# siyi-wind/MDViT

Hardware: AMD Instinct MI355X
Metric: 512x512 images/sec MDViT train step (fwd+bwd, two-sweep, AdamW) (higher is better)
Workload: dtype bf16x3 (fp32 storage; GEMM operands split hi+lo bf16, fp32 accumulate); 1 GPU; MDViT Sup+MLPFM train step, 4 domain(s) x bs=4 per GPU, 512x512, drop_rate=0.1 drop_path=0.1, bf16x3 GEMMs, data-parallel x1

## Files before the change

### include/mdvit_hip.h

```cpp
#ifndef MDVIT_HIP_H
#define MDVIT_HIP_H

#include <stddef.h>
#include <stdint.h>

#ifdef __cplusplus
extern "C" {
#endif

#define MDVIT_ABI_VERSION 1

enum {
    MDVIT_OK = 0,
    MDVIT_E_SHAPE = 1,
    MDVIT_E_DTYPE = 2,
    MDVIT_E_ALIGN = 3,
    MDVIT_E_WORKSPACE = 4,
    MDVIT_E_HIP = 5
};

enum { MDVIT_EPI_NONE = 0, MDVIT_EPI_GELU_DUAL = 1, MDVIT_EPI_DGELU = 2 };
enum { MDVIT_ACT_NONE = 0, MDVIT_ACT_HSWISH = 1, MDVIT_ACT_RELU = 2 };

const char* mdvit_last_error(void);
// ... 182 lines not shown
int mdvit_layernorm_fwd(const float* x, const float* gamma, const float* beta, float* y, float* mean, float* rstd,
                        int32_t M, int32_t C, int32_t groups, float eps, void* stream);
int mdvit_layernorm_bwd(const float* dy, const float* x, const float* gamma, const float* mean, const float* rstd,
                        const float* add, float* dx, float* dgamma, float* dbeta, void* ws , size_t ws_bytes,
                        int32_t M, int32_t C, int32_t groups, void* stream);
int mdvit_layernorm_bwd_masked(const float* dy, const float* x, const float* gamma, const float* mean, const float* rstd, const float* add, float* dx,
                               float* dx_masked, float* dgamma, float* dbeta, void* ws, size_t ws_bytes, int32_t M, int32_t C, int32_t groups,
                               float drop_p, uint32_t key0, uint32_t key1, const float* rowscale, int32_t rows_per_scale, const uint32_t* seed, void* stream);

int mdvit_dwconv3x3_fwd(const float* x, const float* w, const float* bias, float* y,
                        int32_t B, int32_t Hi, int32_t Wi, int32_t C, int32_t stride, int32_t add_input, void* stream);
int mdvit_dwconv3x3_bwd(const float* dy, const float* x, const float* w, float* dx, float* dw, float* dbias,
                        void* ws , size_t ws_bytes,
                        int32_t B, int32_t Hi, int32_t Wi, int32_t C, int32_t stride, int32_t add_input,
                        int32_t accumulate , void* stream);
int mdvit_gconv2_3x3_fwd(const float* skip, const float* up, const float* w, float* y,
                         int32_t B, int32_t H, int32_t W, int32_t C, void* stream);
int mdvit_gconv2_3x3_bwd(const float* dy, const float* skip, const float* up, const float* w,
                         float* dskip, float* dup, float* dw, void* ws , size_t ws_bytes,
                         int32_t B, int32_t H, int32_t W, int32_t C, int32_t accumulate , void* stream);
int mdvit_im2col3x3(const float* x, float* col, int32_t B, int32_t Hi, int32_t Wi, int32_t Cin, int32_t stride, int32_t dilation, void* stream);
int mdvit_col2im3x3(const float* dcol, float* dx, int32_t B, int32_t Hi, int32_t Wi, int32_t Cin, int32_t stride, int32_t dilation, void* stream);
int mdvit_dropout_f32(const float* x, float* y, int64_t n, float p, uint32_t key0, uint32_t key1, const uint32_t* drop_seed, void* stream);
int mdvit_stemconv_fwd(const float* img, const float* w, float* y, int32_t B, int32_t H, int32_t W, int32_t Cin, int32_t Cout, void* stream);
int mdvit_stemconv_wgrad(const float* img, const float* dy, float* dw, void* ws , size_t ws_bytes,
                         int32_t B, int32_t H, int32_t W, int32_t Cin, int32_t Cout, int32_t accumulate , void* stream);

size_t mdvit_bn_ws_bytes(int32_t M, int32_t C, int32_t groups);
int mdvit_bn_stats(const float* y, void* ws, size_t ws_bytes, float* mean, float* rstd, float* running_mean, float* running_var,
                   int64_t* num_batches_tracked, int32_t M, int32_t C, int32_t groups, int32_t per_group_affine, float eps,
                   float momentum, void* stream);
int mdvit_bn_eval_prep(const float* running_mean, const float* running_var, float* mean, float* rstd, int32_t C, float eps, void* stream);
int mdvit_bn_apply(const float* y, const float* mean, const float* rstd, const float* gamma, const float* beta, float* z,
                   int32_t M, int32_t C, int32_t groups, int32_t per_group_affine, int32_t act, float drop2d_p, uint32_t key0,
                   uint32_t key1, const uint32_t* drop_seed, int32_t rows_per_sample, void* stream);
int mdvit_bn_bwd(const float* dz, const float* y, const float* mean, const float* rstd, const float* gamma, const float* beta,
                 float* dy, float* dgamma, float* dbeta, void* ws, size_t ws_bytes, int32_t M, int32_t C, int32_t groups,
                 int32_t per_group_affine, int32_t act, int32_t training, float drop2d_p, uint32_t key0, uint32_t key1, const uint32_t* drop_seed, int32_t rows_per_sample,
                 void* stream);

size_t mdvit_bn_rowdot_ws_bytes(int32_t M, int32_t C);
int mdvit_bn_rowdot_fwd(const float* y, const float* mean, const float* rstd, const float* gamma, const float* beta, const float* w, const float* b ,
                        float* low, int32_t M, int32_t C, int32_t act, float drop2d_p, uint32_t key0, uint32_t key1, const uint32_t* drop_seed,
                        int32_t rows_per_sample, void* stream);
int mdvit_bn_rowdot_bwd(const float* g, const float* y, const float* mean, const float* rstd, const float* gamma, const float* beta, const float* w,
                        float* dy, float* dgamma, float* dbeta, float* dw, float* db , void* ws, size_t ws_bytes, int32_t M, int32_t C, int32_t act,
                        int32_t training, float drop2d_p, uint32_t key0, uint32_t key1, const uint32_t* drop_seed, int32_t rows_per_sample, void* stream);

int mdvit_upsample_fwd(const float* x, const float* base , float* y,
                       int32_t B, int32_t Hi, int32_t Wi, int32_t Ho, int32_t Wo, int32_t C, void* stream);
size_t mdvit_upsample_bwd_ws_bytes(int32_t B, int32_t Hi, int32_t Wi, int32_t Ho, int32_t Wo, int32_t C);
int mdvit_upsample_bwd(const float* dy, float* dx, void* ws, size_t ws_bytes, int32_t B, int32_t Hi, int32_t Wi, int32_t Ho, int32_t Wo,
                       int32_t C, void* stream);

int mdvit_upsample_multi_fwd(const float* const* xs, const int32_t* Hi, const int32_t* Wi, int32_t n, const float* base, float* y, int32_t B, int32_t Ho,
                             int32_t Wo, int32_t C, void* stream);
size_t mdvit_upsample_multi_bwd_ws_bytes(const int32_t* Wi, int32_t n, int32_t B, int32_t Ho, int32_t C);
int mdvit_upsample_multi_bwd(const float* dy, float* const* dxs, const int32_t* Hi, const int32_t* Wi, int32_t n, void* ws, size_t ws_bytes, int32_t B,
                             int32_t Ho, int32_t Wo, int32_t C, void* stream);

int mdvit_da_fwd(const float* label, const float* W1, const float* b1, const float* W2, const float* b2, float* a,
                 int32_t B, int32_t D, int32_t hid, int32_t C, int32_t heads, void* stream);
#define MDVIT_DA_MANY_MAX 32
typedef struct MdvitDaMany {
    int32_t n;
    int32_t hid[MDVIT_DA_MANY_MAX], C[MDVIT_DA_MANY_MAX], heads[MDVIT_DA_MANY_MAX];
    const float* W1[MDVIT_DA_MANY_MAX]; const float* b1[MDVIT_DA_MANY_MAX]; const float* W2[MDVIT_DA_MANY_MAX]; const float* b2[MDVIT_DA_MANY_MAX];
    float* a[MDVIT_DA_MANY_MAX];
} MdvitDaMany;
int mdvit_da_fwd_many(const MdvitDaMany* m, const float* label, int32_t B, int32_t D, void* stream);
typedef struct MdvitDaManyGrads {
    const float* e[MDVIT_DA_MANY_MAX];
    float* dW1[MDVIT_DA_MANY_MAX]; float* db1[MDVIT_DA_MANY_MAX]; float* dW2[MDVIT_DA_MANY_MAX]; float* db2[MDVIT_DA_MANY_MAX];
} MdvitDaManyGrads;
size_t mdvit_da_many_ws_bytes(const MdvitDaMany* m, int32_t B);
int mdvit_da_bwd_many(const MdvitDaMany* m, const MdvitDaManyGrads* g, const float* label, float scale, void* ws, size_t ws_bytes, int32_t B, int32_t D, void* stream);
size_t mdvit_da_ws_bytes(int32_t B, int32_t hid, int32_t C);
int mdvit_da_bwd(const float* label, const float* W1, const float* b1, const float* W2, const float* b2, const float* a,
                 const float* e, float scale, float* dW1, float* db1, float* dW2, float* db2, void* ws, size_t ws_bytes,
                 int32_t B, int32_t D, int32_t hid, int32_t C, int32_t heads, void* stream);

size_t mdvit_factoratt_ws_bytes(int32_t B, int32_t N, int32_t C, int32_t heads);
int mdvit_factoratt_fwd(const float* qkv, const float* w3, const float* b3, const float* w5, const float* b5,
                        const float* w7, const float* b7, const float* a, float* out, float* U, float* kmax, float* ksum, float* Mmat,
                        void* ws, size_t ws_bytes, int32_t B, int32_t H, int32_t W, int32_t C, int32_t heads,
                        int32_t s3, int32_t s5, int32_t s7, void* stream);
int mdvit_factoratt_bwd(const float* dout, const float* qkv, const float* out, const float* U,
                        const float* w3, const float* b3, const float* w5, const float* b5, const float* w7, const float* b7,
                        const float* a, const float* kmax, const float* ksum, const float* Mmat,
                        float* dqkv, float* e, float* dw3, float* db3, float* dw5, float* db5, float* dw7, float* db7,
                        void* ws, size_t ws_bytes, int32_t B, int32_t H, int32_t W, int32_t C, int32_t heads,
                        int32_t s3, int32_t s5, int32_t s7, void* stream);
int mdvit_factoratt_wgrad(const float* qkv, void* ws, size_t ws_bytes, float* dw3, float* db3, float* dw5, float* db5,
                          float* dw7, float* db7, int32_t B, int32_t H, int32_t W, int32_t C, int32_t heads,
                          int32_t s3, int32_t s5, int32_t s7, int32_t accumulate, void* stream);

int mdvit_seg_losses_fwd(const float* out, const float* aux, const float* label, double* sums, float* losses, int64_t n, void* stream);
int mdvit_seg_losses_sums(const float* out, const float* aux, const float* label, double* sums, int64_t n, void* stream);
int mdvit_seg_losses_final(const double* sums, float* losses, int64_t n_total, int32_t has_aux, void* stream);
int mdvit_seg_losses_bwd(const float* out, const float* aux, const float* label, const double* sums, const float* g,
                         float* dout, float* daux, int64_t n, float dice_gain, void* stream);
int mdvit_seg_losses_bwd3(const float* out, const float* aux, const float* label, const double* sums, const float* g0, const float* g1, const float* g2,
                          float* dout, float* daux, int64_t n, float dice_gain, void* stream);
int mdvit_seg_losses_groups_sums(const float* out, const float* aux, const float* label, double* sums, int64_t n, int32_t G, void* stream);
int mdvit_seg_losses_groups_final(const double* sums, float* losses, float* per_group, int64_t n_total, int32_t has_aux, int32_t G, void* stream);
int mdvit_seg_losses_groups_bwd(const float* out, const float* aux, const float* label, const double* sums, const float* g0, const float* g1, const float* g2,
// ... 69 lines not shown
```

### mdvit_amd/_lib.py

```python
from __future__ import annotations

import ctypes as C
import os
import re
from typing import List

_HERE = os.path.dirname(os.path.abspath(__file__))
LIB_PATH = os.environ.get("MDVIT_HIP_LIB") or os.path.join(_HERE, "lib", "libmdvit_hip.so")
HEADER_PATH = os.path.join(_HERE, "..", "include", "mdvit_hip.h")

EPI_NONE, EPI_GELU_DUAL, EPI_DGELU = 0, 1, 2
ACT_NONE, ACT_HSWISH, ACT_RELU = 0, 1, 2

f32p = C.c_void_p
vp = C.c_void_p
i32 = C.c_int32
i64 = C.c_int64
u32 = C.c_uint32
f32 = C.c_float


class GemmDesc(C.Structure):
    _fields_ = [
        ("A", vp), ("B", vp), ("C", vp), ("C2", vp),
# ... 145 lines not shown
    "mdvit_patchify": [vp, vp, i32, i32, i32, i32, i32, vp],
    "mdvit_dropout2d": [vp, vp, i32, i64, i32, f32, u32, u32, vp, vp],
    "mdvit_sdpa_fwd": [vp, vp, vp, vp, i32, i32, i32, i32, vp],
    "mdvit_sdpa_bwd": [vp, vp, vp, vp, vp, vp, vp, vp, i32, i32, i32, i32, vp],
    "mdvit_sdpa_mfma_fwd": [vp, vp, vp, vp, i32, i32, i32, i32, vp],
    "mdvit_sdpa_mfma_bwd": [vp, vp, vp, vp, vp, vp, vp, vp, i32, i32, i32, i32, vp],
    "mdvit_structure_weight": [vp, vp, vp, i32, i32, i32, vp],
    "mdvit_structure_loss_fwd": [vp, vp, vp, vp, vp, i32, i64, vp],
    "mdvit_structure_loss_bwd": [vp, vp, vp, vp, vp, vp, i32, i64, vp],
    "mdvit_split_planes": [vp, i64, vp, i64, i64, i64, i32, i32, vp],
    "mdvit_split_planes_many": [vp, i32, i32, i32, vp],
    "mdvit_split_planes_t": [vp, i64, vp, i64, i64, i32, i32, i32, i32, vp],
    "mdvit_event_create": [C.POINTER(vp)],
    "mdvit_event_destroy": [vp],
    "mdvit_event_elapsed_ms": [vp, vp, C.POINTER(f32)],
    "mdvit_timing_arm": [vp, vp],
    "mdvit_gemm_f32": [C.POINTER(GemmDesc), vp],
    "mdvit_gemm_plan": [C.POINTER(GemmDesc), C.POINTER(i32), C.POINTER(i32), C.POINTER(i32)],
    "mdvit_gemm_force_plan": [i32, i32],
    "mdvit_conv_weight_relayout": [vp, vp, i32, i32, i32, vp],
    "mdvit_conv_weight_relayout_many": [vp, i32, i32, vp],
    "mdvit_gemm_kernel_name": [vp, C.c_char_p, i32],
    "mdvit_gemm_tn_config": [i32, i32, i32],
    "mdvit_gemm_tn_grid_order": [i32],
    "mdvit_transpose_f32": [vp, i64, vp, i32, i32, vp],
    "mdvit_mlp_bwd_dgrad_f32": [vp, vp, vp, vp, vp, vp, vp, vp, i32, i32, i32, f32, u32, u32, vp, vp],
    "mdvit_mlp_fwd_f32": [vp, vp, vp, vp, vp, vp, vp, i32, vp, vp, i32, i32, i32, f32, u32, u32, u32, u32, vp, vp],
    "mdvit_transpose_many": [vp, i32, i32, vp],
    "mdvit_rowdot_fwd": [vp, i64, vp, vp, vp, i32, i32, i32, vp],
    "mdvit_rowdot_bwd": [vp, i64, vp, vp, vp, i64, vp, vp, vp, C.c_size_t, i32, i32, vp],
    "mdvit_colsum_f32": [vp, i64, vp, vp, vp, C.c_size_t, i32, i32, f32, u32, u32, vp, i32, i32, vp, vp],
    "mdvit_layernorm_fwd": [vp, vp, vp, vp, vp, vp, i32, i32, i32, f32, vp],
    "mdvit_layernorm_bwd": [vp, vp, vp, vp, vp, vp, vp, vp, vp, vp, C.c_size_t, i32, i32, i32, vp],
    "mdvit_layernorm_bwd_masked": [vp, vp, vp, vp, vp, vp, vp, vp, vp, vp, vp, C.c_size_t, i32, i32, i32, f32, u32, u32, vp, i32, vp, vp],
    "mdvit_dwconv3x3_fwd": [vp, vp, vp, vp, i32, i32, i32, i32, i32, i32, vp],
    "mdvit_dwconv3x3_bwd": [vp, vp, vp, vp, vp, vp, vp, C.c_size_t, i32, i32, i32, i32, i32, i32, i32, vp],
    "mdvit_gconv2_3x3_fwd": [vp, vp, vp, vp, i32, i32, i32, i32, vp],
    "mdvit_gconv2_3x3_bwd": [vp, vp, vp, vp, vp, vp, vp, vp, C.c_size_t, i32, i32, i32, i32, i32, vp],
    "mdvit_im2col3x3": [vp, vp, i32, i32, i32, i32, i32, i32, vp],
    "mdvit_col2im3x3": [vp, vp, i32, i32, i32, i32, i32, i32, vp],
    "mdvit_dropout_f32": [vp, vp, i64, f32, u32, u32, vp, vp],
    "mdvit_stemconv_fwd": [vp, vp, vp, i32, i32, i32, i32, i32, vp],
    "mdvit_stemconv_wgrad": [vp, vp, vp, vp, C.c_size_t, i32, i32, i32, i32, i32, i32, vp],
    "mdvit_bn_rowdot_fwd": [vp, vp, vp, vp, vp, vp, vp, vp, i32, i32, i32, f32, u32, u32, vp, i32, vp],
    "mdvit_bn_rowdot_bwd": [vp, vp, vp, vp, vp, vp, vp, vp, vp, vp, vp, vp, vp, C.c_size_t, i32, i32, i32, i32, f32, u32, u32, vp, i32, vp],
    "mdvit_bn_stats": [vp, vp, C.c_size_t, vp, vp, vp, vp, vp, i32, i32, i32, i32, f32, f32, vp],
    "mdvit_bn_eval_prep": [vp, vp, vp, vp, i32, f32, vp],
    "mdvit_bn_apply": [vp, vp, vp, vp, vp, vp, i32, i32, i32, i32, i32, f32, u32, u32, vp, i32, vp],
    "mdvit_bn_bwd": [vp, vp, vp, vp, vp, vp, vp, vp, vp, vp, C.c_size_t, i32, i32, i32, i32, i32, i32, f32, u32, u32, vp, i32, vp],
    "mdvit_upsample_multi_fwd": [vp, vp, vp, i32, vp, vp, i32, i32, i32, i32, vp],
    "mdvit_upsample_multi_bwd": [vp, vp, vp, vp, i32, vp, C.c_size_t, i32, i32, i32, i32, vp],
    "mdvit_upsample_fwd": [vp, vp, vp, i32, i32, i32, i32, i32, i32, vp],
    "mdvit_upsample_bwd": [vp, vp, vp, C.c_size_t, i32, i32, i32, i32, i32, i32, vp],
    "mdvit_da_fwd": [vp, vp, vp, vp, vp, vp, i32, i32, i32, i32, i32, vp],
    "mdvit_da_bwd": [vp] * 7 + [f32] + [vp] * 4 + [vp, C.c_size_t] + [i32] * 5 + [vp],
    "mdvit_factoratt_fwd": [vp] * 13 + [vp, C.c_size_t] + [i32] * 8 + [vp],
    "mdvit_factoratt_wgrad": [vp, vp, C.c_size_t] + [vp] * 6 + [i32] * 9 + [vp],
    "mdvit_factoratt_bwd": [vp] * 22 + [vp, C.c_size_t] + [i32] * 8 + [vp],
    "mdvit_seg_losses_fwd": [vp, vp, vp, vp, vp, i64, vp],
    "mdvit_adamw_step": [vp, i32, i32, vp, vp, f32, f32, f32, f32, i32, vp],
    "mdvit_seg_metrics": [vp, vp, vp, vp, vp, i64, vp],
    "mdvit_image_normalize_u8": [vp, vp, i32, i32, i32, vp],
    "mdvit_augment_normalize_u8": [vp, vp, vp, vp, vp, vp, i32, i32, i32, vp],
    "mdvit_augment_probe_taps": [f32, f32, i32, i32, C.POINTER(i32), C.POINTER(f32)],
    "mdvit_seg_losses_sums": [vp, vp, vp, vp, i64, vp],
    "mdvit_seg_losses_final": [vp, vp, i64, i32, vp],
    "mdvit_seg_losses_bwd": [vp, vp, vp, vp, vp, vp, vp, i64, f32, vp],
    "mdvit_seg_losses_bwd3": [vp, vp, vp, vp, vp, vp, vp, vp, vp, i64, f32, vp],
    "mdvit_seg_losses_groups_sums": [vp, vp, vp, vp, i64, i32, vp],
    "mdvit_seg_losses_groups_final": [vp, vp, vp, i64, i32, i32, vp],
    "mdvit_seg_losses_groups_bwd": [vp, vp, vp, vp, vp, vp, vp, vp, vp, i64, i32, f32, vp],
    "mdvit_se_adapter_fwd": [C.POINTER(SeAdapterDesc), vp, vp, vp, vp, C.c_size_t, vp],
    "mdvit_se_adapter_bwd": [C.POINTER(SeAdapterDesc)] + [vp] * 10 + [vp, C.c_size_t, vp],
}

_lib = None


class MdvitHipError(RuntimeError):
    pass


def declared_symbols() -> List[str]:
    with open(HEADER_PATH) as f:
        text = f.read()
    text = re.sub(r"/\*.*?\*/", "", text, flags=re.S)
    return sorted(set(re.findall(r"\b(mdvit_[a-z0-9_]+)\s*\(", text)))


_on_load = []


def on_load(fn):
    if _lib is not None:
        fn(_lib)
    else:
        _on_load.append(fn)


def load():
    global _lib
    if _lib is not None:
        return _lib
    if not os.path.exists(LIB_PATH):
        raise MdvitHipError(
            f"{LIB_PATH} is missing: build it with `python -m mdvit_amd.build` (hipcc, gfx950). "
# ... 71 lines not shown
```

### mdvit_amd/csrc/conv.hip

```cpp
#include "common.h"
#include "conv_tile.h"

namespace {

__device__ __forceinline__ float4 f4_fma(float4 a, float4 w, float4 acc) {
    acc.x = fmaf(a.x, w.x, acc.x); acc.y = fmaf(a.y, w.y, acc.y); acc.z = fmaf(a.z, w.z, acc.z); acc.w = fmaf(a.w, w.w, acc.w);
    return acc;
}
__device__ __forceinline__ float4 f4_add(float4 a, float4 b) { return make_float4(a.x + b.x, a.y + b.y, a.z + b.z, a.w + b.w); }

__global__ __launch_bounds__(256) void dwconv3x3_fwd_kernel(const float* __restrict__ x, const float* __restrict__ w,
                                                            const float* __restrict__ bias, float* __restrict__ y,
                                                            int B, int Hi, int Wi, int C, int stride, int add_input) {
    extern __shared__ float s_w[];
    for (int i = threadIdx.x; i < 9 * C; i += blockDim.x) { const int c = i / 9, t = i % 9; s_w[t * C + c] = w[i]; }
    __syncthreads();
    const int Ho = (Hi - 1) / stride + 1, Wo = (Wi - 1) / stride + 1, QC = C >> 2;
    const long total = (long)B * Ho * Wo * QC;
    for (long e = (long)blockIdx.x * blockDim.x + threadIdx.x; e < total; e += (long)gridDim.x * blockDim.x) {
        const int c = (int)(e % QC) * 4;
        long tkn = e / QC;
        const int wo = (int)(tkn % Wo); tkn /= Wo;
        const int ho = (int)(tkn % Ho);
        const int b = (int)(tkn / Ho);
// ... 701 lines not shown
        if (j >= p.Wi[0]) { j -= p.Wi[0]; src = 1; if (j >= p.Wi[1]) { j -= p.Wi[1]; src = 2; } }
        const int Wi = p.Wi[src];
        const float sc = (float)Wi / (float)Wo;
        int lo, hi;
        out_range(j, Wi, Wo, lo, hi);
        float4 acc = make_float4(0.f, 0.f, 0.f, 0.f);
        const float* base = dy + o * Wo * C + c;
#pragma unroll 4
        for (int t = lo; t < hi; ++t) {
            int i0, i1; float l;
            bilin_src(t, Wi, sc, i0, i1, l);
            const float wgt = (i0 == j ? 1.f - l : 0.f) + (i1 == j ? l : 0.f);
            const float4 g = *reinterpret_cast<const float4*>(base + (long)t * C);
            acc.x = fmaf(wgt, g.x, acc.x); acc.y = fmaf(wgt, g.y, acc.y); acc.z = fmaf(wgt, g.z, acc.z); acc.w = fmaf(wgt, g.w, acc.w);
        }
        float* dsts[3] = {p.d[0], p.d[1], p.d[2]};
        *reinterpret_cast<float4*>(dsts[src] + (o * Wi + j) * C + c) = acc;
    }
}

__global__ __launch_bounds__(256) void upsample_multi_bwd_w_lds_kernel(UpMulti p, const float* __restrict__ dy, int Wo, int C) {
    extern __shared__ __attribute__((aligned(16))) float s_row[];
    const long o = blockIdx.x;
    const int c0 = blockIdx.y * 32;
    const float* src = dy + o * Wo * C + c0;
    for (int e = threadIdx.x; e < Wo * 8; e += 256) {
        const int t = e >> 3, q = e & 7;
        *reinterpret_cast<float4*>(s_row + t * 32 + 4 * q) = *reinterpret_cast<const float4*>(src + (long)t * C + 4 * q);
    }
    __syncthreads();
    const int Wsum = p.Wi[0] + (p.n > 1 ? p.Wi[1] : 0) + (p.n > 2 ? p.Wi[2] : 0);
    float* dsts[3] = {p.d[0], p.d[1], p.d[2]};
    for (int e = threadIdx.x; e < Wsum * 8; e += 256) {
        const int q = e & 7;
        int j = e >> 3, sidx = 0;
        if (j >= p.Wi[0]) { j -= p.Wi[0]; sidx = 1; if (j >= p.Wi[1]) { j -= p.Wi[1]; sidx = 2; } }
        const int Wi = p.Wi[sidx];
        const float sc = (float)Wi / (float)Wo;
        int lo, hi;
        out_range(j, Wi, Wo, lo, hi);
        float4 acc = make_float4(0.f, 0.f, 0.f, 0.f);
#pragma unroll 4
        for (int t = lo; t < hi; ++t) {
            int i0, i1; float l;
            bilin_src(t, Wi, sc, i0, i1, l);
            const float wgt = (i0 == j ? 1.f - l : 0.f) + (i1 == j ? l : 0.f);
            const float4 g = *reinterpret_cast<const float4*>(s_row + t * 32 + 4 * q);
            acc.x = fmaf(wgt, g.x, acc.x); acc.y = fmaf(wgt, g.y, acc.y); acc.z = fmaf(wgt, g.z, acc.z); acc.w = fmaf(wgt, g.w, acc.w);
        }
        *reinterpret_cast<float4*>(dsts[sidx] + (o * Wi + j) * C + c0 + 4 * q) = acc;
    }
}

__global__ __launch_bounds__(256) void dropout_kernel(const float* __restrict__ x, float* __restrict__ y, long n4, uint32_t k0, uint32_t k1,
                                                      const uint32_t* __restrict__ seed, uint32_t thresh, float inv_keep) {
    const uint32_t k0e = k0 ^ (seed ? seed[0] : 0u), k1e = k1 + (seed ? seed[1] : 0u);
    for (long i = (long)blockIdx.x * blockDim.x + threadIdx.x; i < n4; i += (long)gridDim.x * blockDim.x) {
        const float4 v = *reinterpret_cast<const float4*>(x + 4 * i);
        const float4 d = mdvit_drop_scale4(k0e, k1e, (uint32_t)(4 * i), thresh, inv_keep);
        *reinterpret_cast<float4*>(y + 4 * i) = make_float4(v.x * d.x, v.y * d.y, v.z * d.z, v.w * d.w);
    }
}

inline int ew_grid(long total) { return (int)min((total + 255) / 256, 16384L); }

}

extern "C" int mdvit_dwconv3x3_fwd(const float* x, const float* w, const float* bias, float* y, int32_t B, int32_t Hi, int32_t Wi,
                                   int32_t C, int32_t stride, int32_t add_input, void* stream) {
    MDVIT_CHECK_ARG(B > 0 && Hi > 0 && Wi > 0 && C > 0 && C % 4 == 0 && C <= 4096, MDVIT_E_SHAPE, "dwconv3x3_fwd: bad shape B=%d H=%d W=%d C=%d", B, Hi, Wi, C);
    MDVIT_CHECK_ARG(stride == 1 || stride == 2, MDVIT_E_SHAPE, "dwconv3x3_fwd: stride must be 1 or 2");
    MDVIT_CHECK_ARG(!(add_input && stride != 1), MDVIT_E_SHAPE, "dwconv3x3_fwd: add_input needs stride 1");
    const int Ho = (Hi - 1) / stride + 1, Wo = (Wi - 1) / stride + 1;
    if (stride == 1) {
        launch_conv_tile<3, false>(x, (long)C, 0, w, bias, y, (long)C, 0, CtGeom{B, Hi, Wi}, C, (hipStream_t)stream, add_input);
        MDVIT_LAUNCH_CHECK();
        return MDVIT_OK;
    }
    const long total = (long)B * Ho * Wo * C / 4;
    hipLaunchKernelGGL(dwconv3x3_fwd_kernel, dim3(ew_grid(total)), dim3(256), sizeof(float) * 9 * C, (hipStream_t)stream,
                       x, w, bias, y, B, Hi, Wi, C, stride, add_input);
    MDVIT_LAUNCH_CHECK();
    return MDVIT_OK;
}

extern "C" int mdvit_dwconv3x3_bwd(const float* dy, const float* x, const float* w, float* dx, float* dw, float* dbias, void* ws, size_t ws_bytes,
                                   int32_t B, int32_t Hi, int32_t Wi, int32_t C, int32_t stride, int32_t add_input, int32_t accumulate,
                                   void* stream) {
    hipStream_t s = (hipStream_t)stream;
    MDVIT_CHECK_ARG(B > 0 && Hi > 0 && Wi > 0 && C > 0 && C % 4 == 0 && C <= 1024, MDVIT_E_SHAPE, "dwconv3x3_bwd: bad shape B=%d H=%d W=%d C=%d", B, Hi, Wi, C);
    MDVIT_CHECK_ARG(stride == 1 || stride == 2, MDVIT_E_SHAPE, "dwconv3x3_bwd: stride must be 1 or 2");
    const int Ho = (Hi - 1) / stride + 1, Wo = (Wi - 1) / stride + 1;
    if (stride == 1) {
        const CtGeom cg{B, Hi, Wi};
        if (dx) launch_conv_tile<3, true>(dy, (long)C, 0, w, nullptr, dx, (long)C, 0, cg, C, s, add_input);
        if (dw) {
            int tpb; long nblk;
            conv_wgrad_plan(cg, C, tpb, nblk);
            MDVIT_CHECK_PARTIALS_WS(ws, ws_bytes, nblk, CT_CL * 10, "dwconv3x3_bwd");
            const int rc = launch_conv_tile_wgrad<3>(dy, (long)C, 0, x, (long)C, 0, dw, dbias, (float*)ws, cg, C, s, accumulate);
            if (rc != MDVIT_OK) return rc;
        }
        MDVIT_LAUNCH_CHECK();
        return MDVIT_OK;
    }
    if (dx) {
// ... 78 lines not shown
    MDVIT_CHECK_ARG(n > 0 && n % 4 == 0 && n < (1L << 32) && p >= 0.f && p < 1.f, MDVIT_E_SHAPE, "dropout: need 0 < n < 2^32, n %% 4 == 0, 0 <= p < 1 (n=%ld p=%g)", (long)n, p);
    MDVIT_CHECK_ARG(aligned16(x) && aligned16(y), MDVIT_E_ALIGN, "dropout: 16-byte aligned buffers");
    hipLaunchKernelGGL(dropout_kernel, dim3(ew_grid(n / 4)), dim3(256), 0, (hipStream_t)stream, x, y, (long)(n / 4), key0, key1, drop_seed,
                       mdvit_drop_thresh(p), 1.f / (1.f - p));
    MDVIT_LAUNCH_CHECK();
    return MDVIT_OK;
}

extern "C" int mdvit_stemconv_fwd(const float* img, const float* w, float* y, int32_t B, int32_t H, int32_t W, int32_t Cin, int32_t Cout, void* stream) {
    MDVIT_CHECK_ARG(Cin == 3, MDVIT_E_SHAPE, "stemconv_fwd: only in_chans == 3 is built (got %d)", Cin);
    MDVIT_CHECK_ARG(B > 0 && H > 0 && W > 0 && Cout > 0 && Cout % 4 == 0 && Cout <= 256, MDVIT_E_SHAPE, "stemconv_fwd: bad shape");
    const int Ho = (H - 1) / 2 + 1, Wo = (W - 1) / 2 + 1;
    static const bool px32 = [] { const char* e = getenv("MDVIT_STEM_FWD32"); return !(e && e[0] == '0'); }();
    if (px32 && Cout == 32)
        hipLaunchKernelGGL((stemconv_fwd32_kernel<3>), dim3((int)min(((long)B * Ho * Wo + 127) / 128, 8192L)), dim3(256), 0, (hipStream_t)stream, img, w, y, B, H, W);
    else
        hipLaunchKernelGGL((stemconv_fwd_kernel<3>), dim3(ew_grid((long)B * Ho * Wo * Cout / 4)), dim3(256), sizeof(float) * 27 * Cout, (hipStream_t)stream,
                           img, w, y, B, H, W, Cout);
    MDVIT_LAUNCH_CHECK();
    return MDVIT_OK;
}

extern "C" int mdvit_stemconv_wgrad(const float* img, const float* dy, float* dw, void* ws, size_t ws_bytes, int32_t B, int32_t H, int32_t W,
                                    int32_t Cin, int32_t Cout, int32_t accumulate, void* stream) {
    hipStream_t s = (hipStream_t)stream;
    MDVIT_CHECK_ARG(Cin == 3, MDVIT_E_SHAPE, "stemconv_wgrad: only in_chans == 3 is built (got %d)", Cin);
    MDVIT_CHECK_ARG(B > 0 && H > 0 && W > 0 && Cout > 0 && Cout <= 256, MDVIT_E_SHAPE, "stemconv_wgrad: bad shape");
    const int Ho = (H - 1) / 2 + 1, Wo = (W - 1) / 2 + 1;
    const long npix = (long)B * Ho * Wo;
    int ppb = (int)max(64L, (npix + 2047) / 2048);
    const int nblk = cdiv(npix, ppb);
    MDVIT_CHECK_PARTIALS_WS(ws, ws_bytes, nblk, 27 * Cout, "stemconv_wgrad");
    static const bool mfma = [] { const char* e = getenv("MDVIT_STEM_WGRAD_MFMA"); return !(e && e[0] == '0'); }();
    if (mfma && Cout % 32 == 0) {
        ppb = (int)max(128L, (npix + 1023) / 1024);
        const int nb2 = cdiv(npix, ppb);
        hipLaunchKernelGGL((stemconv_wgrad_mfma_kernel<3>), dim3(nb2), dim3(256), 0, s, img, dy, (float*)ws, B, H, W, Cout, ppb);
        MDVIT_LAUNCH_CHECK();
        return mdvit_reduce_partials((const float*)ws, nb2, 27L * Cout, 27 * Cout, dw, 0, nullptr, accumulate, s);
    }
    hipLaunchKernelGGL((stemconv_wgrad_kernel<3>), dim3(nblk), dim3(256), sizeof(float) * 27 * Cout, s, img, dy, (float*)ws, B, H, W, Cout, ppb);
    MDVIT_LAUNCH_CHECK();
    return mdvit_reduce_partials((const float*)ws, nblk, 27L * Cout, 27 * Cout, dw, 0, nullptr, accumulate, s);
}

extern "C" int mdvit_upsample_fwd(const float* x, const float* base, float* y, int32_t B, int32_t Hi, int32_t Wi, int32_t Ho, int32_t Wo, int32_t C, void* stream) {
    MDVIT_CHECK_ARG(B > 0 && Hi > 0 && Wi > 0 && Ho > 0 && Wo > 0 && C > 0, MDVIT_E_SHAPE, "upsample_fwd: bad shape");
    const long total = (long)B * Ho * Wo * ((C & 3) == 0 ? C / 4 : C);
    hipLaunchKernelGGL(upsample_fwd_kernel, dim3(ew_grid(total)), dim3(256), 0, (hipStream_t)stream, x, base, y, B, Hi, Wi, Ho, Wo, C);
    MDVIT_LAUNCH_CHECK();
    return MDVIT_OK;
}

extern "C" size_t mdvit_upsample_bwd_ws_bytes(int32_t B, int32_t Hi, int32_t Wi, int32_t Ho, int32_t Wo, int32_t C) {
    if (B <= 0 || Hi <= 0 || Wi <= 0 || Ho <= 0 || Wo <= 0 || C <= 0) return 0;
    return sizeof(float) * (size_t)B * Ho * Wi * C;
}

extern "C" int mdvit_upsample_bwd(const float* dy, float* dx, void* ws, size_t ws_bytes, int32_t B, int32_t Hi, int32_t Wi, int32_t Ho, int32_t Wo,
                                  int32_t C, void* stream) {
    hipStream_t s = (hipStream_t)stream;
    MDVIT_CHECK_ARG(B > 0 && Hi > 0 && Wi > 0 && Ho > 0 && Wo > 0 && C > 0, MDVIT_E_SHAPE, "upsample_bwd: bad shape");
    MDVIT_CHECK_ARG(ws != nullptr && ws_bytes >= mdvit_upsample_bwd_ws_bytes(B, Hi, Wi, Ho, Wo, C), MDVIT_E_WORKSPACE,
                    "upsample_bwd: workspace too small (mdvit_upsample_bwd_ws_bytes)");
    float* tmp = (float*)ws;
    const int vec = (C & 3) == 0 && aligned16(dy) && aligned16(dx) && aligned16(tmp);
    const long cq = vec ? C / 4 : C;
    {
        const long total = (long)B * Ho * Wi * cq;
        hipLaunchKernelGGL((upsample_bwd_pass_kernel<true>), dim3(ew_grid(total)), dim3(256), 0, s, dy, tmp, (long)B * Ho, Wi, Wo, cq, vec);
    }
    {
        const long total = (long)B * Hi * Wi * cq;
        hipLaunchKernelGGL((upsample_bwd_pass_kernel<false>), dim3(ew_grid(total)), dim3(256), 0, s, tmp, dx, (long)B, Hi, Ho, (long)Wi * cq, vec);
    }
    MDVIT_LAUNCH_CHECK();
    return MDVIT_OK;
}

extern "C" int mdvit_upsample_multi_fwd(const float* const* xs, const int32_t* Hi, const int32_t* Wi, int32_t n, const float* base, float* y, int32_t B, int32_t Ho,
                                        int32_t Wo, int32_t C, void* stream) {
    MDVIT_CHECK_ARG(n >= 1 && n <= 3 && B > 0 && Ho > 0 && Wo > 0 && C > 0 && C % 4 == 0, MDVIT_E_SHAPE, "upsample_multi_fwd: 1..3 sources, C %% 4 == 0 (n=%d C=%d)", n, C);
    UpMulti p; memset(&p, 0, sizeof(p));
    p.n = n;
    for (int i = 0; i < n; ++i) {
        MDVIT_CHECK_ARG(xs[i] && Hi[i] > 0 && Wi[i] > 0 && aligned16(xs[i]), MDVIT_E_SHAPE, "upsample_multi_fwd: bad source %d", i);
        p.x[i] = xs[i]; p.Hi[i] = Hi[i]; p.Wi[i] = Wi[i];
    }
    MDVIT_CHECK_ARG(aligned16(y) && (!base || aligned16(base)), MDVIT_E_ALIGN, "upsample_multi_fwd: y / base must be 16-byte aligned");
    {
        bool ok = Ho % UT_H == 0 && Wo % UT_W == 0 && C % UT_C == 0 && (long)(Ho / UT_H) * (Wo / UT_W) < (1L << 30) && C / UT_C < 65536 && B < 65536;
        int pool = 0;
        for (int i = 0; i < n && ok; ++i) {
            const int fh = Ho / Hi[i], fw = Wo / Wi[i];
            ok = Ho % Hi[i] == 0 && Wo % Wi[i] == 0 && fh >= 2 && fw >= 2 && fh <= 16 && fw <= 16 && (fh & (fh - 1)) == 0 && (fw & (fw - 1)) == 0;
            if (ok) pool += (UT_H / fh + 2) * (UT_W / fw + 2);
        }
        if (ok && pool <= UT_POOL) {
            hipLaunchKernelGGL(upsample_multi_tile_kernel, dim3((Ho / UT_H) * (Wo / UT_W), C / UT_C, B), dim3(256), 0, (hipStream_t)stream, p, base, y, Ho, Wo, C);
            MDVIT_LAUNCH_CHECK();
            return MDVIT_OK;
        }
    }
    MDVIT_CHECK_ARG((long)Wo * (C / 4) < (1L << 30), MDVIT_E_SHAPE, "upsample_multi_fwd: output row too long");
    const long nunits = (long)B * Ho * (((long)Wo * (C / 4) + 1023) >> 10);
    hipLaunchKernelGGL(upsample_multi_fwd_kernel, dim3((unsigned)min(nunits, 16384L)), dim3(256), 0, (hipStream_t)stream, p, base, y, B, Ho, Wo, C);
    MDVIT_LAUNCH_CHECK();
    return MDVIT_OK;
}

extern "C" size_t mdvit_upsample_multi_bwd_ws_bytes(const int32_t* Wi, int32_t n, int32_t B, int32_t Ho, int32_t C) {
    size_t t = 0;
    for (int i = 0; i < n && i < 3; ++i) t += (size_t)B * Ho * Wi[i] * C;
    return sizeof(float) * t;
}

extern "C" int mdvit_upsample_multi_bwd(const float* dy, float* const* dxs, const int32_t* Hi, const int32_t* Wi, int32_t n, void* ws, size_t ws_bytes, int32_t B,
                                        int32_t Ho, int32_t Wo, int32_t C, void* stream) {
    hipStream_t s = (hipStream_t)stream;
    MDVIT_CHECK_ARG(n >= 1 && n <= 3 && B > 0 && Ho > 0 && Wo > 0 && C > 0 && C % 4 == 0, MDVIT_E_SHAPE, "upsample_multi_bwd: 1..3 sources, C %% 4 == 0 (n=%d C=%d)", n, C);
    MDVIT_CHECK_ARG(ws && ws_bytes >= mdvit_upsample_multi_bwd_ws_bytes(Wi, n, B, Ho, C) && aligned16(ws) && aligned16(dy), MDVIT_E_WORKSPACE,
                    "upsample_multi_bwd: workspace too small (mdvit_upsample_multi_bwd_ws_bytes)");
    UpMulti p; memset(&p, 0, sizeof(p));
    p.n = n;
    float* t = (float*)ws;
    int wsum = 0;
    for (int i = 0; i < n; ++i) {
        MDVIT_CHECK_ARG(dxs[i] && Hi[i] > 0 && Wi[i] > 0 && aligned16(dxs[i]), MDVIT_E_SHAPE, "upsample_multi_bwd: bad source %d", i);
        p.Hi[i] = Hi[i]; p.Wi[i] = Wi[i]; p.d[i] = t;
        t += (size_t)B * Ho * Wi[i] * C;
        wsum += Wi[i];
    }
    const long cq = C / 4;
    const int bpr = (int)cdiv((long)wsum * cq, 256L);
    MDVIT_CHECK_ARG((long)B * Ho * bpr < (1L << 31), MDVIT_E_SHAPE, "upsample_multi_bwd: too many workgroups");
    if (C % 32 == 0 && Wo <= 384 && (long)B * Ho < (1L << 31) && C / 32 <= 65535)
        hipLaunchKernelGGL(upsample_multi_bwd_w_lds_kernel, dim3((unsigned)((long)B * Ho), C / 32), dim3(256), sizeof(float) * Wo * 32, s, p, dy, Wo, C);
    else
        hipLaunchKernelGGL(upsample_multi_bwd_w_kernel, dim3((unsigned)((long)B * Ho * bpr)), dim3(256), 0, s, p, dy, (long)B * Ho, Wo, C, bpr);
    for (int i = 0; i < n; ++i)
        hipLaunchKernelGGL((upsample_bwd_pass_kernel<false>), dim3(ew_grid((long)B * Hi[i] * Wi[i] * cq)), dim3(256), 0, s, p.d[i], dxs[i], (long)B, Hi[i], Ho,
                           (long)Wi[i] * cq, 1);
    MDVIT_LAUNCH_CHECK();
    return MDVIT_OK;
}
```

### mdvit_amd/ops.py

```python
from __future__ import annotations

import ctypes as C
import itertools
import os
import weakref
from typing import Optional, Tuple

import torch

from . import _lib
from ._lib import GemmDesc, call

_key_counter = itertools.count(1)
_POISON = os.environ.get("MDVIT_POISON", "0") == "1"


def _empty(*a, **k):
    t = torch.empty(*a, **k)
    if _POISON and t.is_floating_point():
        t.fill_(float("nan"))
    return t


def _empty_like(x):
# ... 1931 lines not shown
            off += n
        return tuple(out)

    @staticmethod
    def backward(ctx, *gs):
        if all(g is None for g in gs):
            return None, None
        ref = next(g for g in gs if g is not None)
        parts = [g if g is not None else torch.zeros((ctx.rows, n), device=ref.device, dtype=ref.dtype) for g, n in zip(gs, ctx.sizes)]
        return torch.cat(parts, 1), None


class _CatChannels(torch.autograd.Function):

    @staticmethod
    def forward(ctx, a, b):
        ctx.set_materialize_grads(False)
        ctx.sizes = (a.shape[-1], b.shape[-1])
        return torch.cat([a, b], dim=-1)

    @staticmethod
    def backward(ctx, g):
        if g is None:
            return None, None
        c0, _c1 = ctx.sizes
        return (g[..., :c0].contiguous() if ctx.needs_input_grad[0] else None), (g[..., c0:].contiguous() if ctx.needs_input_grad[1] else None)


def cat_channels(a, b):
    return _CatChannels.apply(_c(a), _c(b))


def split_cols(W, sizes):
    assert W.dim() == 2 and sum(sizes) == W.shape[1]
    return _SplitCols.apply(W, tuple(int(n) for n in sizes))


def split_groups(x, groups: int):
    if groups == 1:
        return (x,)
    assert x.shape[0] % groups == 0
    return _SplitGroups.apply(_c(x), int(groups))


def bn_act(y, gamma, beta, running_mean, running_var, nbt, training, act, eps=1e-5, momentum=0.1, drop2d_p=0.0):
    rows_per_sample = y.numel() // (y.shape[0] * y.shape[-1])
    groups = _bn_groups if (training or gamma.dim() == 2) else 1
    if groups > 1 and y.shape[0] % groups:
        raise ValueError(f"bn_groups({groups}) needs a batch that is a multiple of it, got {y.shape[0]}")
    return _BNAct.apply(_c(y), _c(gamma), _c(beta), running_mean, running_var, nbt, bool(training), float(eps), float(momentum),
                        int(act), float(drop2d_p), int(rows_per_sample), int(groups))


class _Upsample(torch.autograd.Function):
    @staticmethod
    def forward(ctx, x, Ho, Wo, base):
        ctx.set_materialize_grads(False)
        _chk(x, base)
        B, H, W_, Cn = x.shape
        y = _empty((B, Ho, Wo, Cn), device=x.device, dtype=torch.float32)
        call("mdvit_upsample_fwd", _p(x), _p(base), _p(y), B, H, W_, Ho, Wo, Cn, _stream())
        ctx.meta = (B, H, W_, Ho, Wo, Cn, base is not None)
        return y

    @staticmethod
    def backward(ctx, g):
        if g is None:
            return (None,) * 4
        B, H, W_, Ho, Wo, Cn, has_base = ctx.meta
        g = _c(g)
        dx = _empty((B, H, W_, Cn), device=g.device, dtype=torch.float32)
        wsb = _lib.load().mdvit_upsample_bwd_ws_bytes(B, H, W_, Ho, Wo, Cn)
        ws = _empty((wsb // 4,), device=g.device, dtype=torch.float32)
        call("mdvit_upsample_bwd", _p(g), _p(dx), _p(ws), wsb, B, H, W_, Ho, Wo, Cn, _stream())
        return dx, None, None, (g if has_base else None)


def upsample_bilinear(x, Ho, Wo, base=None):
    if base is None and x.shape[1] == Ho and x.shape[2] == Wo:
        return x
    return _Upsample.apply(_c(x), int(Ho), int(Wo), None if base is None else _c(base))


class _UpsampleSum(torch.autograd.Function):

    @staticmethod
    def forward(ctx, base, Ho, Wo, *xs):
        ctx.set_materialize_grads(False)
        _chk(base, *xs)
        B, _, _, Cn = xs[0].shape
        n = len(xs)
        y = _empty((B, Ho, Wo, Cn), device=xs[0].device, dtype=torch.float32)
        ptrs = (C.c_void_p * n)(*[x.data_ptr() for x in xs])
        Hi = (C.c_int32 * n)(*[x.shape[1] for x in xs])
        Wi = (C.c_int32 * n)(*[x.shape[2] for x in xs])
        call("mdvit_upsample_multi_fwd", ptrs, Hi, Wi, n, _p(base), _p(y), B, Ho, Wo, Cn, _stream())
        ctx.meta = (B, Ho, Wo, Cn, [(x.shape[1], x.shape[2]) for x in xs], base is not None)
        return y

    @staticmethod
    def backward(ctx, g):
        B, Ho, Wo, Cn, dims, has_base = ctx.meta
        if g is None:
            return (None,) * (3 + len(dims))
        g = _c(g)
        n = len(dims)
# ... 817 lines not shown
```

Before: 516.3 images/s.

## Fuse bilinear upsample backward width and height passes into single kernels

Adds a fused multi-source upsample backward kernel that streams dy rows through double-buffered LDS, applies precomputed width weights and accumulates height contributions in registers, writing dx directly instead of going through a workspace and a second height pass. Also adds a simple fused single-source kernel for small-channel upsample backward. Both apply only to even integer scale factors and are on by default, with an env switch to disable. The goal is to remove the intermediate workspace round trip and extra launches, at the cost of complex indexing and possible lower occupancy from LDS use.

```diff
diff --git a/include/mdvit_hip.h b/include/mdvit_hip.h
--- a/include/mdvit_hip.h
+++ b/include/mdvit_hip.h
@@ -258,6 +258,7 @@
 size_t mdvit_upsample_bwd_ws_bytes(int32_t B, int32_t Hi, int32_t Wi, int32_t Ho, int32_t Wo, int32_t C);
 int mdvit_upsample_bwd(const float* dy, float* dx, void* ws, size_t ws_bytes, int32_t B, int32_t Hi, int32_t Wi, int32_t Ho, int32_t Wo,
                        int32_t C, void* stream);
+int mdvit_upsample_bwd_config(int32_t fused);
 
 int mdvit_upsample_multi_fwd(const float* const* xs, const int32_t* Hi, const int32_t* Wi, int32_t n, const float* base, float* y, int32_t B, int32_t Ho,
                              int32_t Wo, int32_t C, void* stream);
diff --git a/mdvit_amd/_lib.py b/mdvit_amd/_lib.py
--- a/mdvit_amd/_lib.py
+++ b/mdvit_amd/_lib.py
@@ -221,6 +221,7 @@
     "mdvit_upsample_multi_bwd": [vp, vp, vp, vp, i32, vp, C.c_size_t, i32, i32, i32, i32, vp],
     "mdvit_upsample_fwd": [vp, vp, vp, i32, i32, i32, i32, i32, i32, vp],
     "mdvit_upsample_bwd": [vp, vp, vp, C.c_size_t, i32, i32, i32, i32, i32, i32, vp],
+    "mdvit_upsample_bwd_config": [i32],
     "mdvit_da_fwd": [vp, vp, vp, vp, vp, vp, i32, i32, i32, i32, i32, vp],
     "mdvit_da_bwd": [vp] * 7 + [f32] + [vp] * 4 + [vp, C.c_size_t] + [i32] * 5 + [vp],
     "mdvit_factoratt_fwd": [vp] * 13 + [vp, C.c_size_t] + [i32] * 8 + [vp],
diff --git a/mdvit_amd/csrc/conv.hip b/mdvit_amd/csrc/conv.hip
--- a/mdvit_amd/csrc/conv.hip
+++ b/mdvit_amd/csrc/conv.hip
@@ -777,6 +777,206 @@
     }
 }
 
+constexpr int UA_R = 16;
+constexpr int UA_ITEMS = 4;
+constexpr int UA_PAD = 8;
+constexpr int UA_HT = UA_R + 32;
+
+template <int NPF>
+__global__ __launch_bounds__(256) void upsample_multi_bwd_fused_kernel(UpMulti p, const float* __restrict__ dy, int Ho, int Wo, int C) {
+    extern __shared__ __attribute__((aligned(16))) float s_rows[];
+    const int rowf = (Wo + 2 * UA_PAD) * 32;
+    float4* s_ht = reinterpret_cast<float4*>(s_rows + 2 * rowf);
+    float* s_wt = reinterpret_cast<float*>(s_ht + UA_HT * 3);
+    const int c0 = blockIdx.x * 32, b = blockIdx.z;
+    const int R0 = blockIdx.y * UA_R, R1 = min(R0 + UA_R, Ho);
+    int ob = Ho, oe = 0;
+    for (int i = 0; i < p.n; ++i) {
+        const int s = Ho / p.Hi[i];
+        const int rf = (R0 + s - 1) / s, re = min(p.Hi[i], (R1 + s - 1) / s);
+        if (rf < re) { ob = min(ob, max(0, s * rf - s / 2)); oe = max(oe, min(Ho, s * (re - 1) + 3 * s / 2)); }
+    }
+    if (ob >= oe) return;
+    for (int e = threadIdx.x; e < (oe - ob) * p.n; e += 256) {
+        const int o = ob + e / p.n, i = e % p.n;
+        const int Hi = i == 0 ? p.Hi[0] : i == 1 ? p.Hi[1] : p.Hi[2];
+        const int s = Ho / Hi, rh = (o + s / 2) / s;
+        int i0, i1; float l;
+        bilin_src(o, Hi, (float)Hi / (float)Ho, i0, i1, l);
+        const int rE = (rh & 1) ? rh - 1 : rh, rO = (rh & 1) ? rh : rh - 1;
+        const float wE = (i0 == rE ? 1.f - l : 0.f) + (i1 == rE ? l : 0.f);
+        const float wO = (i0 == rO ? 1.f - l : 0.f) + (i1 == rO ? l : 0.f);
+        int ev = 0;
+        if ((o + 1 + s / 2) % s == 0) {
+            const int rd = rh - 1, rf = (R0 + s - 1) / s, re = min(Hi, (R1 + s - 1) / s);
+            ev = 2 * (rd + 2) + (rd >= rf && rd < re ? 1 : 0);
+        }
+        s_ht[(o - ob) * 3 + i] = make_float4(wE, wO, __int_as_float(ev), 0.f);
+    }
+    {
+        int wbase = 0;
+        for (int i = 0; i < p.n; ++i) {
+            const int Wi = p.Wi[i], s = Wo / Wi;
+            const float sc = (float)Wi / (float)Wo;
+            for (int e = threadIdx.x; e < Wi * 2 * s; e += 256) {
+                const int j = e / (2 * s), t = s * j - s / 2 + e % (2 * s);
+                float wgt = 0.f;
+                if (t >= 0 && t < Wo) {
+                    int i0, i1; float l;
+                    bilin_src(t, Wi, sc, i0, i1, l);
+                    wgt = (i0 == j ? 1.f - l : 0.f) + (i1 == j ? l : 0.f);
+                }
+                s_wt[wbase + e] = wgt;
+            }
+            wbase += Wi * 2 * s;
+        }
+    }
+    for (int e = threadIdx.x; e < 2 * 2 * UA_PAD * 8; e += 256) {
+        const int buf = e / (2 * UA_PAD * 8), r = e % (2 * UA_PAD * 8), px = r >> 3;
+        *reinterpret_cast<float4*>(s_rows + buf * rowf + (px < UA_PAD ? px : Wo + px) * 32 + 4 * (r & 7)) = make_float4(0.f, 0.f, 0.f, 0.f);
+    }
+    const int Wsum = p.Wi[0] + (p.n > 1 ? p.Wi[1] : 0) + (p.n > 2 ? p.Wi[2] : 0);
+    const int q = threadIdx.x & 7;
+    int it_src[UA_ITEMS], it_t0[UA_ITEMS], it_s2[UA_ITEMS], it_wo[UA_ITEMS];
+    long it_rs[UA_ITEMS];
+    float* it_dx[UA_ITEMS];
+    float4 aE[UA_ITEMS], aO[UA_ITEMS];
+#pragma unroll
+    for (int k = 0; k < UA_ITEMS; ++k) {
+        const int e = threadIdx.x + 256 * k;
+        int j = e >> 3, sidx = 0, wbase = 0;
+        if (j >= p.Wi[0]) {
+            j -= p.Wi[0]; sidx = 1; wbase = 2 * Wo;
+            if (j >= p.Wi[1]) { j -= p.Wi[1]; sidx = 2; wbase = 4 * Wo; }
+        }
+        if (e >= Wsum * 8) { sidx = -1; j = 0; }
+        const int Hi = sidx <= 0 ? p.Hi[0] : sidx == 1 ? p.Hi[1] : p.Hi[2];
+        const int Wi = sidx <= 0 ? p.Wi[0] : sidx == 1 ? p.Wi[1] : p.Wi[2];
+        float* dx = sidx <= 0 ? p.d[0] : sidx == 1 ? p.d[1] : p.d[2];
+        const int s = Wo / Wi;
+        it_src[k] = sidx;
+        it_t0[k] = s * j - s / 2 + UA_PAD; it_s2[k] = 2 * s;
+        it_wo[k] = wbase + j * 2 * s;
+        it_rs[k] = (long)Wi * C;
+        it_dx[k] = dx + ((long)b * Hi * Wi + j) * C + c0 + 4 * q;
+        aE[k] = make_float4(0.f, 0.f, 0.f, 0.f); aO[k] = make_float4(0.f, 0.f, 0.f, 0.f);
+    }
+    const float* src = dy + (long)b * Ho * Wo * C + c0;
+    typedef float f4v __attribute__((ext_vector_type(4)));
+    f4v pfa[NPF], pfb[NPF];
+#pragma unroll
+    for (int u = 0; u < NPF; ++u) {
+        const int e = threadIdx.x + 256 * u;
+        if (e < Wo * 8) *reinterpret_cast<float4*>(s_rows + (UA_PAD + (e >> 3)) * 32 + 4 * (e & 7)) = *reinterpret_cast<const float4*>(src + ((long)ob * Wo + (e >> 3)) * C + 4 * (e & 7));
+    }
+#define UA_FMA(wv, gv) acc.x = fmaf(wv, gv.x, acc.x); acc.y = fmaf(wv, gv.y, acc.y); acc.z = fmaf(wv, gv.z, acc.z); acc.w = fmaf(wv, gv.w, acc.w);
+#define UA_STEP(o, cur, ld, st) { \
+        { \
+        _Pragma("unroll") \
+            for (int u = 0; u < NPF; ++u) { \
+                const int e = min((int)threadIdx.x + 256 * u, Wo * 8 - 1); \
+                ld[u] = *reinterpret_cast<const f4v*>(src + ((long)min(o + 2, oe - 1) * Wo + (e >> 3)) * C + 4 * (e & 7)); \
+            } \
+        } \
+        const float* s_row = s_rows + cur * rowf + 4 * q; \
+        _Pragma("unroll") \
+        for (int k = 0; k < UA_ITEMS; ++k) { \
+            if (it_src[k] < 0 || (o) >= oe) continue; \
+            const float* wt = s_wt + it_wo[k]; \
+            const float* sr = s_row + it_t0[k] * 32; \
+            float4 acc = make_float4(0.f, 0.f, 0.f, 0.f); \
+            int u = 0; \
+            for (; u + 8 <= it_s2[k]; u += 8) { \
+                const float4 w0 = *reinterpret_cast<const float4*>(wt + u), w1 = *reinterpret_cast<const float4*>(wt + u + 4); \
+                const float4 g0 = *reinterpret_cast<const float4*>(sr + (u + 0) * 32), g1 = *reinterpret_cast<const float4*>(sr + (u + 1) * 32); \
+                const float4 g2 = *reinterpret_cast<const float4*>(sr + (u + 2) * 32), g3 = *reinterpret_cast<const float4*>(sr + (u + 3) * 32); \
+                const float4 g4 = *reinterpret_cast<const float4*>(sr + (u + 4) * 32), g5 = *reinterpret_cast<const float4*>(sr + (u + 5) * 32); \
+                const float4 g6 = *reinterpret_cast<const float4*>(sr + (u + 6) * 32), g7 = *reinterpret_cast<const float4*>(sr + (u + 7) * 32); \
+                UA_FMA(w0.x, g0) UA_FMA(w0.y, g1) UA_FMA(w0.z, g2) UA_FMA(w0.w, g3) UA_FMA(w1.x, g4) UA_FMA(w1.y, g5) UA_FMA(w1.z, g6) UA_FMA(w1.w, g7) \
+            } \
+            if (u < it_s2[k]) { \
+                const float4 w0 = *reinterpret_cast<const float4*>(wt + u); \
+                const float4 g0 = *reinterpret_cast<const float4*>(sr + (u + 0) * 32), g1 = *reinterpret_cast<const float4*>(sr + (u + 1) * 32); \
+                const float4 g2 = *reinterpret_cast<const float4*>(sr + (u + 2) * 32), g3 = *reinterpret_cast<const float4*>(sr + (u + 3) * 32); \
+                UA_FMA(w0.x, g0) UA_FMA(w0.y, g1) UA_FMA(w0.z, g2) UA_FMA(w0.w, g3) \
+            } \
+            const float4 h = s_ht[(o - ob) * 3 + it_src[k]]; \
+            aE[k].x = fmaf(h.x, acc.x, aE[k].x); aE[k].y = fmaf(h.x, acc.y, aE[k].y); aE[k].z = fmaf(h.x, acc.z, aE[k].z); aE[k].w = fmaf(h.x, acc.w, aE[k].w); \
+            aO[k].x = fmaf(h.y, acc.x, aO[k].x); aO[k].y = fmaf(h.y, acc.y, aO[k].y); aO[k].z = fmaf(h.y, acc.z, aO[k].z); aO[k].w = fmaf(h.y, acc.w, aO[k].w); \
+            const int ev = __float_as_int(h.z); \
+            if (ev) { \
+                const int rd = (ev >> 1) - 2; \
+                float* d = it_dx[k] + rd * it_rs[k]; \
+                if (rd & 1) { if (ev & 1) *reinterpret_cast<float4*>(d) = aO[k]; aO[k] = make_float4(0.f, 0.f, 0.f, 0.f); } \
+                else        { if (ev & 1) *reinterpret_cast<float4*>(d) = aE[k]; aE[k] = make_float4(0.f, 0.f, 0.f, 0.f); } \
+            } \
+        } \
+        if (o + 1 < oe) { \
+            float* nxt = s_rows + (cur ^ 1) * rowf + UA_PAD * 32; \
+        _Pragma("unroll") \
+            for (int u = 0; u < NPF; ++u) { \
+                const int e = threadIdx.x + 256 * u; \
+                if (e < Wo * 8) *reinterpret_cast<f4v*>(nxt + (e >> 3) * 32 + 4 * (e & 7)) = st[u]; \
+            } \
+        } \
+        __syncthreads(); \
+    }
+#pragma unroll
+    for (int u = 0; u < NPF; ++u) {
+        const int e = min((int)threadIdx.x + 256 * u, Wo * 8 - 1);
+        pfb[u] = *reinterpret_cast<const f4v*>(src + ((long)min(ob + 1, Ho - 1) * Wo + (e >> 3)) * C + 4 * (e & 7));
+    }
+    __syncthreads();
+    for (int o = ob; o < oe; o += 2) {
+        UA_STEP(o, 0, pfa, pfb)
+        UA_STEP(o + 1, 1, pfb, pfa)
+    }
+#undef UA_STEP
+#undef UA_FMA
+#pragma unroll
+    for (int k = 0; k < UA_ITEMS; ++k) {
+        if (it_src[k] < 0) continue;
+        const int Hi = it_src[k] == 0 ? p.Hi[0] : it_src[k] == 1 ? p.Hi[1] : p.Hi[2];
+        const int s = Ho / Hi, rh = (oe + s / 2) / s;
+        const int rf = (R0 + s - 1) / s, re = min(Hi, (R1 + s - 1) / s);
+        const int rE = (rh & 1) ? rh - 1 : rh, rO = (rh & 1) ? rh : rh - 1;
+        if (rE >= rf && rE < re) *reinterpret_cast<float4*>(it_dx[k] + rE * it_rs[k]) = aE[k];
+        if (rO >= rf && rO < re) *reinterpret_cast<float4*>(it_dx[k] + rO * it_rs[k]) = aO[k];
+    }
+}
+
+__global__ __launch_bounds__(256) void upsample_bwd_fused_kernel(const float* __restrict__ dy, float* __restrict__ dx, int B, int Hi, int Wi, int Ho, int Wo, int C) {
+    const float sch = (float)Hi / (float)Ho, scw = (float)Wi / (float)Wo;
+    const long total = (long)B * Hi * Wi * C;
+    for (long e = (long)blockIdx.x * blockDim.x + threadIdx.x; e < total; e += (long)gridDim.x * blockDim.x) {
+        const int c = (int)(e % C);
+        long r = e / C;
+        const int j = (int)(r % Wi); r /= Wi;
+        const int i = (int)(r % Hi);
+        const long b = r / Hi;
+        int lo_h, hi_h, lo_w, hi_w;
+        out_range(i, Hi, Ho, lo_h, hi_h);
+        out_range(j, Wi, Wo, lo_w, hi_w);
+        float acc = 0.f;
+        for (int o = lo_h; o < hi_h; ++o) {
+            const float* base = dy + (b * Ho + o) * Wo * C + c;
+            float tw = 0.f;
+#pragma unroll 4
+            for (int t = lo_w; t < hi_w; ++t) {
+                int i0, i1; float l;
+                bilin_src(t, Wi, scw, i0, i1, l);
+                const float wgt = (i0 == j ? 1.f - l : 0.f) + (i1 == j ? l : 0.f);
+                tw = fmaf(wgt, base[(long)t * C], tw);
+            }
+            int i0, i1; float l;
+            bilin_src(o, Hi, sch, i0, i1, l);
+            const float wgt = (i0 == i ? 1.f - l : 0.f) + (i1 == i ? l : 0.f);
+            acc = fmaf(wgt, tw, acc);
+        }
+        dx[e] = acc;
+    }
+}
+
 __global__ __launch_bounds__(256) void dropout_kernel(const float* __restrict__ x, float* __restrict__ y, long n4, uint32_t k0, uint32_t k1,
                                                       const uint32_t* __restrict__ seed, uint32_t thresh, float inv_keep) {
     const uint32_t k0e = k0 ^ (seed ? seed[0] : 0u), k1e = k1 + (seed ? seed[1] : 0u);
@@ -961,6 +1161,13 @@
     return MDVIT_OK;
 }
 
+static int g_upsample_bwd_fused = 1;
+extern "C" int mdvit_upsample_bwd_config(int32_t fused) {
+    g_upsample_bwd_fused = fused != 0;
+    return MDVIT_OK;
+}
+static bool even_factor(int n_in, int n_out) { return n_out % n_in == 0 && ((n_out / n_in) & 1) == 0 && n_out / n_in <= 16; }
+
 extern "C" size_t mdvit_upsample_bwd_ws_bytes(int32_t B, int32_t Hi, int32_t Wi, int32_t Ho, int32_t Wo, int32_t C) {
     if (B <= 0 || Hi <= 0 || Wi <= 0 || Ho <= 0 || Wo <= 0 || C <= 0) return 0;
     return sizeof(float) * (size_t)B * Ho * Wi * C;
@@ -972,6 +1179,11 @@
     MDVIT_CHECK_ARG(B > 0 && Hi > 0 && Wi > 0 && Ho > 0 && Wo > 0 && C > 0, MDVIT_E_SHAPE, "upsample_bwd: bad shape");
     MDVIT_CHECK_ARG(ws != nullptr && ws_bytes >= mdvit_upsample_bwd_ws_bytes(B, Hi, Wi, Ho, Wo, C), MDVIT_E_WORKSPACE,
                     "upsample_bwd: workspace too small (mdvit_upsample_bwd_ws_bytes)");
+    if (g_upsample_bwd_fused && C <= 4 && even_factor(Hi, Ho) && even_factor(Wi, Wo)) {
+        hipLaunchKernelGGL(upsample_bwd_fused_kernel, dim3(ew_grid((long)B * Hi * Wi * C)), dim3(256), 0, s, dy, dx, B, Hi, Wi, Ho, Wo, C);
+        MDVIT_LAUNCH_CHECK();
+        return MDVIT_OK;
+    }
     float* tmp = (float*)ws;
     const int vec = (C & 3) == 0 && aligned16(dy) && aligned16(dx) && aligned16(tmp);
     const long cq = vec ? C / 4 : C;
@@ -1040,6 +1252,19 @@
         t += (size_t)B * Ho * Wi[i] * C;
         wsum += Wi[i];
     }
+    {
+        const size_t lds = sizeof(float) * (2 * ((size_t)Wo + 2 * UA_PAD) * 32 + UA_HT * 3 * 4 + 2 * (size_t)Wo * n);
+        bool ok = g_upsample_bwd_fused && C % 32 == 0 && Wo <= 256 && lds <= 65536 && wsum * 8 <= 256 * UA_ITEMS && B <= 65535 && cdiv((long)Ho, (long)UA_R) <= 65535;
+        for (int i = 0; i < n && ok; ++i) ok = even_factor(Hi[i], Ho) && even_factor(Wi[i], Wo);
+        if (ok) {
+            for (int i = 0; i < n; ++i) p.d[i] = dxs[i];
+            const dim3 grid(C / 32, (unsigned)cdiv((long)Ho, (long)UA_R), B);
+            if (Wo <= 128) hipLaunchKernelGGL((upsample_multi_bwd_fused_kernel<4>), grid, dim3(256), lds, s, p, dy, Ho, Wo, C);
+            else           hipLaunchKernelGGL((upsample_multi_bwd_fused_kernel<8>), grid, dim3(256), lds, s, p, dy, Ho, Wo, C);
+            MDVIT_LAUNCH_CHECK();
+            return MDVIT_OK;
+        }
+    }
     const long cq = C / 4;
     const int bpr = (int)cdiv((long)wsum * cq, 256L);
     MDVIT_CHECK_ARG((long)B * Ho * bpr < (1L << 31), MDVIT_E_SHAPE, "upsample_multi_bwd: too many workgroups");
diff --git a/mdvit_amd/ops.py b/mdvit_amd/ops.py
--- a/mdvit_amd/ops.py
+++ b/mdvit_amd/ops.py
@@ -2007,6 +2007,11 @@
                         int(act), float(drop2d_p), int(rows_per_sample), int(groups))
 
 
+_upsample_bwd_fused = os.environ.get("MDVIT_UPSAMPLE_BWD_FUSED", "1") != "0"
+if not _upsample_bwd_fused:
+    _lib.on_load(lambda lib: lib.mdvit_upsample_bwd_config(0))
+
+
 class _Upsample(torch.autograd.Function):
     @staticmethod
     def forward(ctx, x, Ho, Wo, base):
```

After: 523.6 images/s, median of 6. 1.4% higher.
